# gddickinson/neural_enhanced_super_resolution

Measured on AMD Instinct MI355X. Metric: output megapixels/sec, RealESRGAN_x2plus x2 upscale, higher is better.
Workload: dtype f32 (operands as f16 hi+lo pairs, 3 f16 MFMAs per product, f32 accumulate); 1 GPU; c2: 512x512->1024x1024 RealESRGAN_x2plus fp32 single tile; frames_in_flight_per_gpu=1, world_size=1, partition=independent frames, no data-path collective

## Files before the change

neural_enhanced_super_resolution_amd/csrc/conv3x3_f16x2.hip:

```cpp
#include <cstdlib>
#include <type_traits>

#include "f16x2_common.h"
#include "nesr_kernels.h"

namespace nesr {


namespace {

constexpr int TW = 32, PW = TW + 2;
constexpr int WAVES = 4;
constexpr int RW = 2;

template <int DMAW>
struct Geo {
    static constexpr int LAUNCH_THREADS = 64 * (WAVES + DMAW);
    static constexpr int THREADS = 64 * (DMAW ? DMAW : WAVES);
    static constexpr int TH = WAVES * RW;
    static constexpr int PH = TH + 2;
    static constexpr int NPIX = PH * PW;
    static constexpr int IN_ITEMS = 4 * NPIX;
    static constexpr int IN_ROUNDS = (IN_ITEMS + THREADS - 1) / THREADS;
    static constexpr int IN_BYTES = IN_ITEMS * 16;
// ... 243 lines not shown
            const bool valid = X < a.w_ && Y < y_hi;
            const size_t pix = ((size_t)n * a.h + (Y < a.h ? Y : 0)) * a.w_ + (X < a.w_ ? X : 0);
            f32x4 v0, v1;
#pragma unroll
            for (int i = 0; i < 4; ++i) {
                const float e = fmaf(acc16[r][nh][0][1][i], LO_INV, acc16[r][nh][0][0][i]);
                const float o = fmaf(acc16[r][nh][1][1][i], LO_INV, acc16[r][nh][1][0][i]);
                const auto sw_ = __builtin_amdgcn_permlane16_swap(__float_as_uint(e), __float_as_uint(o), false, false);
                v0[i] = __uint_as_float(sw_[0]);
                v1[i] = __uint_as_float(sw_[1]);
            }
            v0 += bz0;
            v1 += bz1;
            if (a.lrelu) {
#pragma unroll
                for (int i = 0; i < 4; ++i) { v0[i] = fmaxf(v0[i], v0[i] * 0.2f); v1[i] = fmaxf(v1[i], v1[i] * 0.2f); }
            }
            auto slot = [&](const Map& mp, int coff) -> size_t { return (size_t)((coff + 32 * cg) >> 4) * mp.chunk + pix * mp.pix + piece8; };
            if (res1) {
                f32x4 q0, q1;
                load_regrouped(res1 + slot(a.res1_map, 0), a.res1_map.chunk, q0, q1);
#pragma unroll
                for (int i = 0; i < 4; ++i) { v0[i] = __fadd_rn(__fmul_rn(v0[i], a.s1), q0[i]); v1[i] = __fadd_rn(__fmul_rn(v1[i], a.s1), q1[i]); }
            }
            if (res2) {
                f32x4 q0, q1;
                load_regrouped(res2 + slot(a.res2_map, 0), a.res2_map.chunk, q0, q1);
#pragma unroll
                for (int i = 0; i < 4; ++i) { v0[i] = __fadd_rn(__fmul_rn(v0[i], a.s2), q0[i]); v1[i] = __fadd_rn(__fmul_rn(v1[i], a.s2), q1[i]); }
            }
            if (out || out2) {
                uint4 cx, cx1;
                bool bad_here = false;
                split_regroup(v0, v1, cx, cx1, bad_here);
                bad |= bad_here && valid;
                if (valid && out) {
                    uint16_t* p = out + slot(a.out_map, a.out_coff);
                    store16(p, cx);
                    store16(p + a.out_map.chunk, cx1);
                }
                if (valid && out2) {
                    uint16_t* p = out2 + slot(a.out2_map, 0);
                    store16(p, cx);
                    store16(p + a.out2_map.chunk, cx1);
                }
            }
            if (!valid) continue;
            if (a.cout_real > 0 && cb == 0) {
#pragma unroll
                for (int q = 0; q < 4; ++q) {
                    if (q >= a.cout_real) break;
                    const float x = poison ? __builtin_nanf("") : v0[q];
                    if (a.out_nchw) a.out_nchw[(((size_t)n * a.cout_real + q) * a.h + Y) * a.w_ + X] = x;
                    if (a.out_u8) {
                        float qv = fminf(fmaxf(x, 0.f), 1.f) * 255.0f;
                        qv = a.u8_round ? rintf(qv) : truncf(qv);
                        const int ch = a.u8_flip ? (a.cout_real - 1 - q) : q;
                        a.out_u8[pix * a.cout_real + ch] = (uint8_t)qv;
                    }
                }
            }
        }
    if (bad && a.status) __hip_atomic_store(a.status, 1u, __ATOMIC_RELAXED, __HIP_MEMORY_SCOPE_AGENT);
    STAMP(3);
#if NESR_ABL & 64
    asm volatile("s_waitcnt vmcnt(0)" ::: "memory");
    STAMP(4);
#endif
}

struct RdbArgs {
    const void* cur;
    long long chunk_bytes;
    void* out;
    const void* res2;
    float s1, s2;
    const void* w[5];
    const float* bias[5];
    int n, h, w_;
    unsigned* progress;
    unsigned epoch;
    unsigned* abort_flag;
    unsigned* status;
    unsigned long long timeout_ticks;
};

__device__ __forceinline__ void glds16_s_sc1(const char* sbase, unsigned voff, unsigned lds_dst) {
    unsigned keep;
    asm volatile(
        "s_mov_b32 %0, m0\n\t"
        "s_mov_b32 m0, %3\n\t"
        "s_nop 0\n\t"
        "global_load_lds_dwordx4 %1, %2 sc1\n\t"
        "s_mov_b32 m0, %0"
        : "=&s"(keep)
        : "v"(voff), "s"(sbase), "s"(lds_dst)
        : "memory");
}
__device__ __forceinline__ void store16_wt_s(const char* sbase, unsigned voff, uint4 v) {
    asm volatile("global_store_dwordx4 %0, %1, %2 sc1\n\ts_nop 1" ::"v"(voff), "v"(__builtin_bit_cast(f32x4, v)), "s"(sbase) : "memory");
}
__device__ __forceinline__ f32x4 load16_s(const char* sbase, unsigned voff) {
    return *(const __attribute__((address_space(1))) f32x4*)(sbase + voff);
}

#ifndef NESR_RDB_ABL
#define NESR_RDB_ABL 0
#endif

__device__ __forceinline__ void wait_vmcnt_le(int k) {
    switch (k) {
        case 0: asm volatile("s_waitcnt vmcnt(0)" ::: "memory"); break;
        case 1: asm volatile("s_waitcnt vmcnt(1)" ::: "memory"); break;
        case 2: asm volatile("s_waitcnt vmcnt(2)" ::: "memory"); break;
        case 3: asm volatile("s_waitcnt vmcnt(3)" ::: "memory"); break;
        case 4: asm volatile("s_waitcnt vmcnt(4)" ::: "memory"); break;
        case 5: asm volatile("s_waitcnt vmcnt(5)" ::: "memory"); break;
        case 6: asm volatile("s_waitcnt vmcnt(6)" ::: "memory"); break;
        case 7: asm volatile("s_waitcnt vmcnt(7)" ::: "memory"); break;
        case 8: asm volatile("s_waitcnt vmcnt(8)" ::: "memory"); break;
        case 9: asm volatile("s_waitcnt vmcnt(9)" ::: "memory"); break;
        case 10: asm volatile("s_waitcnt vmcnt(10)" ::: "memory"); break;
        case 11: asm volatile("s_waitcnt vmcnt(11)" ::: "memory"); break;
        default: asm volatile("s_waitcnt vmcnt(12)" ::: "memory"); break;
    }
}

#if NESR_RDB_ABL & 256
__device__ unsigned long long g_rdb_stamps[2][64][8];
__device__ unsigned long long g_rdb_taps[2][8][8];
__device__ unsigned long long g_rdb_arrive[12][8][2];
#define RARRIVE(w, step, ev) do { if (blockIdx.x == 77 && lane == 0 && (step) >= 20 && (step) < 28) { unsigned long long t_ = __builtin_amdgcn_s_memtime(); asm volatile("s_waitcnt lgkmcnt(0)" ::: "memory"); g_rdb_arrive[w][(step) - 20][ev] = t_; } } while (0)
#define RSTAMP(role, step, ev) do { if (blockIdx.x == 77 && lane == 0) { unsigned long long t_ = __builtin_amdgcn_s_memtime(); asm volatile("s_waitcnt lgkmcnt(0)" ::: "memory"); g_rdb_stamps[role][step][ev] = t_; } } while (0)
#else
#define RSTAMP(role, step, ev) do { } while (0)
#define RARRIVE(w, step, ev) do { } while (0)
#endif

constexpr int RSLOTS = 4;
constexpr int RDB_STEP5 = 4 + 6 + 8 + 10;
constexpr int RDB_STEPS = RDB_STEP5 + 12;
constexpr int W5_ROUNDS = 2 * W_ITEMS / (64 * 4);
static_assert(RSLOTS == 4 && RDB_STEP5 % RSLOTS == 0 && W5_ROUNDS * 64 * 4 == 2 * W_ITEMS, "conv5's slab pairs sit at ring positions 0,1 / 2,3 and fill whole DMA rounds");
constexpr int MW = 8;
constexpr int DW = 4;
#ifndef NESR_RDB_PAR
#define NESR_RDB_PAR 0
#endif
#ifndef NESR_RDB_EPI_STEPS
#define NESR_RDB_EPI_STEPS 1
#endif
constexpr int EPI_STEPS = NESR_RDB_EPI_STEPS;
static_assert(EPI_STEPS <= 4 - (RSLOTS - 1), "the tile would wait for its own progress word");

__global__ __launch_bounds__(64 * (MW + DW), 3) void rdb_f16x2_kernel(RdbArgs a) {
    typedef Geo<4> G;
    constexpr int THREADS = G::THREADS, TH = G::TH;
    constexpr int IN_ITEMS = G::IN_ITEMS, IN_ROUNDS = G::IN_ROUNDS, IN_BYTES = G::IN_BYTES;
    constexpr int W_ROUNDS = (W_ITEMS + THREADS - 1) / THREADS;
    constexpr int WRING = RSLOTS * IN_BYTES;
    constexpr int BIAS = RSLOTS * (IN_BYTES + W_BYTES);
    static_assert(TH == MW, "one tile row per MFMA wave");
    extern __shared__ __attribute__((aligned(16))) char smem[];

    const int lane = threadIdx.x & 63;
    const int wave_all = __builtin_amdgcn_readfirstlane(threadIdx.x >> 6);
    const bool is_dma = wave_all >= MW;
    const bool is_cmp = !is_dma;
    const int wave = is_cmp ? wave_all : wave_all - MW;
    const int tid = wave * 64 + lane;

    const int tiles_x = (a.w_ + TW - 1) / TW;
    const int tiles_y = (a.h + TH - 1) / TH;
    const int total = tiles_x * tiles_y * a.n;
    int tile;
    {
        const int bid = blockIdx.x, q = total >> 3, r = total & 7, xcd = bid & 7;
        tile = (xcd < r ? xcd * (q + 1) : r * (q + 1) + (xcd - r) * q) + (bid >> 3);
    }
    const int n = tile / (tiles_x * tiles_y);
    const int t2 = tile - n * tiles_x * tiles_y;
    const int ty = t2 / tiles_x, tx = t2 - ty * tiles_x;
    const int y0 = ty * TH, x0 = tx * TW;

    const int j16 = lane & 15, g4 = lane >> 4;
    auto advance = [](int& l, int& c) {
        const int nc = l == 4 ? 12 : 4 + 2 * l;
        if (++c == nc) { c = 0; ++l; }
    };

    if (is_dma) {
#ifdef NESR_RDB_DMAPRIO
        __builtin_amdgcn_s_setprio(NESR_RDB_DMAPRIO);
#endif
        if (wave == 0) RSTAMP(1, 61, 0);
        const unsigned lds_base = (unsigned)(size_t)(lds_char*)(smem);
        unsigned voff[IN_ROUNDS];
        unsigned okmask = 0;
        unsigned wavemask = 0;
        const int row0 = y0 > 0 ? y0 - 1 : 0;
        const char* in_img = static_cast<const char*>(a.cur) + ((size_t)n * a.h + row0) * a.w_ * 64;
        const unsigned* watch = nullptr;
        int kin = 0, kw = 0;
        if (lane < 9) {
            const int ny = ty + lane / 3 - 1, nx = tx + lane % 3 - 1;
            if (ny >= 0 && ny < tiles_y && nx >= 0 && nx < tiles_x) watch = a.progress + (n * tiles_y + ny) * tiles_x + nx;
        }
        {
            int p = tid >> 2;
            int py = p / PW, px = p - py * PW;
            const int sl = tid & 3;
#pragma unroll
            for (int i = 0; i < IN_ROUNDS; ++i) {
                const int k = tid + THREADS * i;
                const int sg = sl ^ (((px >> 2) & 1) << 1);
                const int Y = y0 - 1 + py, X = x0 - 1 + px;
                const bool has = k < IN_ITEMS;
                const bool ok = has && Y >= 0 && Y < a.h && X >= 0 && X < a.w_;
                voff[i] = ((unsigned)(Y - row0) * (unsigned)a.w_ + (unsigned)X) * 64u + sg * 16;
                okmask |= ok ? (1u << i) : 0u;
                if (__builtin_amdgcn_ballot_w64(ok) != 0ull) { wavemask |= 1u << i; ++kin; }
                if (has && !ok) {
#pragma unroll
                    for (int sl2 = 0; sl2 < RSLOTS; ++sl2) *reinterpret_cast<f32x4*>(smem + sl2 * IN_BYTES + k * 16) = f32x4{0.f, 0.f, 0.f, 0.f};
                }
                px += (THREADS / 4) % PW;
                py += (THREADS / 4) / PW;
                if (px >= PW) { px -= PW; py += 1; }
            }
#pragma unroll
            for (int j = 0; j < W_ROUNDS; ++j) kw += (wave * 64 + THREADS * j) < W_ITEMS ? 1 : 0;
        }
        unsigned seen = 0;
        bool gave_up = false;
        auto dma_w = [&](int l, int c, int wpos) {
            const char* wsrc = static_cast<const char*>(a.w[l]) + (size_t)c * W_BYTES;
#pragma unroll
            for (int j = 0; j < W_ROUNDS; ++j) {
                const int k = tid + THREADS * j;
                const unsigned dst = lds_base + WRING + wpos * W_BYTES + j * (THREADS * 16) + wave * 1024;
                if (k < W_ITEMS && !(NESR_RDB_ABL & 64)) glds16_s(wsrc, (unsigned)k * 16u, __builtin_amdgcn_readfirstlane(dst));
            }
        };
        auto dma_w5 = [&](int c, int wpos) {
            const char* wsrc = static_cast<const char*>(a.w[4]) + (size_t)c * (2 * W_BYTES);
#pragma unroll
            for (int j = 0; j < W5_ROUNDS; ++j) {
                const unsigned dst = lds_base + WRING + wpos * W_BYTES + j * (THREADS * 16) + wave * 1024;
                if (!(NESR_RDB_ABL & 64)) glds16_s(wsrc, (unsigned)(tid + THREADS * j) * 16u, __builtin_amdgcn_readfirstlane(dst));
            }
        };
        auto dma_in = [&](int c, int slot) {
            const unsigned need = c < 4 ? 0u : (unsigned)((c - 4) >> 1) + 1u;
            if (need > seen && !gave_up && !(NESR_RDB_ABL & 1)) {
                const unsigned target = a.epoch + need;
                unsigned long long t0 = 0;
                for (unsigned it = 0;; ++it) {
                    const unsigned v = watch ? __hip_atomic_load(watch, __ATOMIC_RELAXED, __HIP_MEMORY_SCOPE_AGENT) : target;
                    if (__builtin_amdgcn_ballot_w64((int)(v - target) < 0) == 0ull) break;
                    if ((it & 63u) == 0u) {
                        const unsigned long long now = __builtin_amdgcn_s_memrealtime();
                        if (it == 0) t0 = now;
                        const unsigned ab = __hip_atomic_load(a.abort_flag, __ATOMIC_RELAXED, __HIP_MEMORY_SCOPE_AGENT);
                        if (ab != 0u || now - t0 > a.timeout_ticks) {
                            if (ab == 0u && lane == 0) __hip_atomic_store(a.abort_flag, 1u | ((unsigned)c << 8) | ((unsigned)tile << 16), __ATOMIC_RELAXED, __HIP_MEMORY_SCOPE_AGENT);
                            gave_up = true;
                            break;
                        }
                    }
                    __builtin_amdgcn_s_sleep(4);
                }
                seen = need;
            }
            const char* isrc = in_img + (long long)c * a.chunk_bytes;
#pragma unroll
            for (int i = 0; i < IN_ROUNDS; ++i) {
                const unsigned dst = lds_base + slot * IN_BYTES + i * (THREADS * 16) + wave * 1024;
                if (((wavemask >> i) & 1u) && !(NESR_RDB_ABL & 32)) {
                    if ((okmask >> i) & 1u) {
                        if (NESR_RDB_ABL & 2) glds16_s(isrc, voff[i], __builtin_amdgcn_readfirstlane(dst));
                        else glds16_s_sc1(isrc, voff[i], __builtin_amdgcn_readfirstlane(dst));
                    }
                }
            }
        };
        int fl = 0, fc = 0;
#pragma unroll
        for (int i = 0; i < RSLOTS - 1; ++i) {
            dma_w(0, i, i);
            dma_in(i, i);
            advance(fl, fc);
        }
        gave_up = *(const __attribute__((address_space(4))) unsigned*)a.abort_flag != 0u;
        asm volatile("s_waitcnt lgkmcnt(0)" ::: "memory");
        int fill = 3;
        int cl = 0, cc = 0;
        wait_vmcnt_le((NESR_RDB_ABL & 96) ? 0 : 2 * (kw + kin));
        int inflight = kw + kin;
        __builtin_amdgcn_s_barrier();
        asm volatile("" ::: "memory");
        for (int step = 0; step < RDB_STEPS; ++step) {
            if (wave == 0) RSTAMP(1, step, 0);
#if NESR_RDB_ABL & 256
            if ((step == 0 || step == RDB_STEPS - 1) && wave == 0 && blockIdx.x == 77 && lane == 0) {
                const unsigned long long r_ = __builtin_amdgcn_s_memrealtime(), t_ = __builtin_amdgcn_s_memtime();
                asm volatile("s_waitcnt lgkmcnt(0)" ::: "memory");
                g_rdb_stamps[1][step == 0 ? 62 : 63][0] = r_;
                g_rdb_stamps[1][step == 0 ? 62 : 63][1] = t_;
            }
#endif
            wait_vmcnt_le((NESR_RDB_ABL & 96) ? 0 : inflight);
            if (wave == 0) RSTAMP(1, step, 1);
            RARRIVE(MW + wave, step, 0);
            if (!(NESR_RDB_ABL & 512)) __builtin_amdgcn_s_barrier();
            asm volatile("" ::: "memory");
            RARRIVE(MW + wave, step, 1);
            if (wave == 0) RSTAMP(1, step, 2);
            if (cc == EPI_STEPS && cl >= 1 && wave == 0 && lane == 0)
                __hip_atomic_store(a.progress + tile, a.epoch + (unsigned)cl, __ATOMIC_RELAXED, __HIP_MEMORY_SCOPE_AGENT);
            inflight = 0;
            if (step + 1 >= RDB_STEP5) {
                if (step + 1 < RDB_STEPS) dma_w5(step + 1 - RDB_STEP5, ((step + 1) & 1) * 2);
            } else if (fl < 4) {
                dma_w(fl, fc, (step + RSLOTS - 1) & (RSLOTS - 1));
                inflight += kw;
            }
            if (fl < 5) {
                dma_in(fc, fill);
                inflight += kin;
                advance(fl, fc);
                fill = fill == RSLOTS - 1 ? 0 : fill + 1;
            }
            if (wave == 0) RSTAMP(1, step, 3);
            advance(cl, cc);
        }
        return;
    }

#ifdef NESR_RDB_YPRIO
    if (wave >= 4) __builtin_amdgcn_s_setprio(NESR_RDB_YPRIO);
#endif
    const bool active = (y0 + wave) < a.h;
    if (wave == 1) RSTAMP(0, 61, 0);
    const bool fills_bias = wave < 6 && lane < 8;
    f32x4 bias_v = f32x4{0.f, 0.f, 0.f, 0.f};
    if (fills_bias) bias_v = *(const __attribute__((address_space(1))) f32x4*)(a.bias[wave < 4 ? wave : 4] + (wave == 5 ? 32 : 0) + 4 * lane);
    const int un = g4 >> 1, kh = g4 & 1;
    int b16[5][2], a16[5];
#pragma unroll
    for (int st_ = 0; st_ < 5; ++st_) {
        const int dy = st_ < 3 ? un : 2;
        const int dx = st_ < 3 ? st_ : (st_ == 3 ? un : 2);
#pragma unroll
        for (int nh = 0; nh < 2; ++nh) {
            const int col = 16 * nh + j16 + dx;
            b16[st_][nh] = ((wave + dy) * PW + col) * 64 + ((kh ^ (((col >> 2) & 1) << 1)) << 4);
        }
        a16[st_] = ((((dy * 3 + dx) * 2) * 2 + kh) * 32 + j16) * 16;
    }
    int slot = 0;
    int wpos = 0;
#if NESR_RDB_ABL & 256
    int mstep = 0;
#endif
    typedef const __attribute__((address_space(3))) f32x4* lds_f32x4;
    const unsigned lds0 = (unsigned)(size_t)(lds_char*)(smem);
    unsigned bcur[5], aw012, aw3, aw4, aw4b;
#pragma unroll
    for (int t = 0; t < 5; ++t) bcur[t] = lds0 + (unsigned)b16[t][0];
    const unsigned xl4 = (unsigned)((un ^ 1) << 5);
    aw012 = lds0 + (unsigned)(WRING + a16[0]);
    aw3 = lds0 + (unsigned)(WRING + a16[3]);
    aw4 = lds0 + (unsigned)(WRING + a16[4]);
    aw4b = aw4 + (unsigned)un * 1024u;
    const int par = (NESR_RDB_PAR >= 0) ? NESR_RDB_PAR : wave >> 2;
    const int cbl = (g4 & 1) * 16 + (g4 >> 1) * 8;
    const int piece8 = ((g4 & 1) * 2 + (g4 >> 1)) * 8;
    const bool res2 = a.res2 != nullptr;
    f32x4 ep[2][2];
#pragma unroll
    for (int nh = 0; nh < 2; ++nh)
#pragma unroll
        for (int mt = 0; mt < 2; ++mt) ep[nh][mt] = f32x4{0.f, 0.f, 0.f, 0.f};
    int ep_l = -1;
    bool bad = false;
    auto unpack_res = [&](f32x4 rx, f32x4 rx1, f32x4& q0, f32x4& q1) {
        uint4 cx = __builtin_bit_cast(uint4, rx), cx1 = __builtin_bit_cast(uint4, rx1);
        regroup_pairs(cx, cx1);
        const f16x8 h = __builtin_bit_cast(f16x8, cx), lo = __builtin_bit_cast(f16x8, cx1);
#pragma unroll
        for (int i = 0; i < 4; ++i) {
            q0[i] = fmaf((float)lo[i], LO_INV, (float)h[i]);
            q1[i] = fmaf((float)lo[4 + i], LO_INV, (float)h[4 + i]);
        }
    };
    const long long row_bytes = (((long long)n * a.h + (y0 + wave)) * a.w_) * 64;
    unsigned lane_off[2];
    bool lane_ok[2];
#pragma unroll
    for (int nh = 0; nh < 2; ++nh) {
        const int X = x0 + 16 * nh + j16;
        lane_ok[nh] = X < a.w_;
        lane_off[nh] = (unsigned)(lane_ok[nh] ? X : 0) * 64u + (unsigned)piece8 * 2u;
    }
    auto uni = [](const char* p) -> const char* {
        const unsigned long long v = (unsigned long long)p;
        const unsigned lo = __builtin_amdgcn_readfirstlane((unsigned)v), hi = __builtin_amdgcn_readfirstlane((unsigned)(v >> 32));
        return (const char*)(((unsigned long long)hi << 32) | lo);
    };
    auto epi_half = [&](int l, const f32x4& e0, const f32x4& e1, int nh) {
#if NESR_RDB_ABL & 256
        if (wave == 1) RSTAMP(0, mstep, 3);
#endif
        const bool valid = lane_ok[nh];
        const unsigned voff = lane_off[nh];
        const char* bsrc = smem + BIAS + (l * 32 + cbl) * 4;
        f32x4 v0, v1;
#pragma unroll
        for (int i = 0; i < 4; ++i) {
            const auto sw_ = __builtin_amdgcn_permlane16_swap(__float_as_uint(e0[i]), __float_as_uint(e1[i]), false, false);
            v0[i] = __uint_as_float(sw_[0]);
            v1[i] = __uint_as_float(sw_[1]);
        }
        v0 += *reinterpret_cast<const f32x4*>(bsrc);
        v1 += *reinterpret_cast<const f32x4*>(bsrc + 16);
        const int dchunk = 4 + 2 * l;
#pragma unroll
        for (int i = 0; i < 4; ++i) { v0[i] = fmaxf(v0[i], v0[i] * 0.2f); v1[i] = fmaxf(v1[i], v1[i] * 0.2f); }
#if NESR_RDB_ABL & 256
        asm volatile("" :: "v"(v0), "v"(v1));
        if (wave == 1) RSTAMP(0, mstep, 4);
#endif
        uint4 cx, cx1;
        bool bad_here = false;
        split_regroup(v0, v1, cx, cx1, bad_here);
        bad |= bad_here && valid;
#if NESR_RDB_ABL & 256
        asm volatile("" :: "v"(__builtin_bit_cast(f32x4, cx)), "v"(__builtin_bit_cast(f32x4, cx1)));
        if (wave == 1) RSTAMP(0, mstep, 5);
#endif
        if (valid) {
            const char* d0 = uni(static_cast<const char*>(a.cur) + (long long)dchunk * a.chunk_bytes + row_bytes);
            if (!(NESR_RDB_ABL & 4)) {
                store16_wt_s(d0, voff, cx);
                store16_wt_s(d0 + a.chunk_bytes, voff, cx1);
            } else {
                *reinterpret_cast<uint4*>(const_cast<char*>(d0) + voff) = cx;
                *reinterpret_cast<uint4*>(const_cast<char*>(d0) + a.chunk_bytes + voff) = cx1;
            }
        }
#if NESR_RDB_ABL & 256
        if (wave == 1) RSTAMP(0, mstep, 6);
#endif
    };
    auto epi_part = [&](int c) {
        if (NESR_RDB_ABL & 16) return;
        if (EPI_STEPS == 1) {
            epi_half(ep_l, ep[0][0], ep[0][1], 0);
            epi_half(ep_l, ep[1][0], ep[1][1], 1);
        } else if (c == 0) {
            epi_half(ep_l, ep[0][0], ep[0][1], 0);
        } else {
            epi_half(ep_l, ep[1][0], ep[1][1], 1);
        }
    };
    f32x4 R1[4][2], R2[4][2];
    auto issue_res = [&](const void* base, int g, f32x4 (&R)[4][2]) {
        const char* r = uni(static_cast<const char*>(base) + (long long)(2 * g) * a.chunk_bytes + row_bytes);
#pragma unroll
        for (int nh = 0; nh < 2; ++nh) {
            R[2 * g + nh][0] = load16_s(r, lane_off[nh]);
            R[2 * g + nh][1] = load16_s(r + a.chunk_bytes, lane_off[nh]);
        }
    };
    f32x4 acc16[2][2][2][2];
    f32x4 Af[2][2][2];
    f32x4 Bf[2][2][2];
    auto load_a = [&](int s_, int buf, unsigned off) {
#pragma unroll
        for (int mt = 0; mt < 2; ++mt) {
            if (s_ < 4) {
                const unsigned ad = s_ < 3 ? aw012 + s_ * 2048 : aw3;
                Af[buf][mt][0] = *((lds_f32x4)(size_t)(ad + off + mt * 256));
                Af[buf][mt][1] = *((lds_f32x4)(size_t)(ad + off + mt * 256 + 1024));
            } else {
                f32x4 hi = *((lds_f32x4)(size_t)(aw4 + off + mt * 256));
                Af[buf][mt][1] = *((lds_f32x4)(size_t)(aw4b + off + mt * 256));
                if (un) hi = f32x4{0.f, 0.f, 0.f, 0.f};
                Af[buf][mt][0] = hi;
            }
        }
    };
    auto move_a = [&](unsigned d) {
        aw012 += d;
        aw3 += d;
        aw4 += d;
        aw4b += d;
    };
    auto load_b = [&](int sl, int s_, int buf) {
        const unsigned dB = sl == RSLOTS - 1 ? (unsigned)(-(RSLOTS - 1) * IN_BYTES) : (unsigned)IN_BYTES;
        const unsigned xl = bcur[s_] ^ (s_ == 4 ? xl4 : 32u);
#pragma unroll
        for (int nh = 0; nh < 2; ++nh) {
            Bf[buf][nh][0] = *((lds_f32x4)(size_t)(bcur[s_] + nh * 1024));
            Bf[buf][nh][1] = *((lds_f32x4)(size_t)(xl + nh * 1024));
        }
        bcur[s_] += dB;
    };
    auto mfma_tap = [&](int s_, int g, int abuf, int bbuf) {
#pragma unroll
        for (int mt = 0; mt < 2; ++mt) {
            const f16x8 a0 = __builtin_bit_cast(f16x8, Af[abuf][mt][0]), a1 = __builtin_bit_cast(f16x8, Af[abuf][mt][1]);
#pragma unroll
            for (int nh = 0; nh < 2; ++nh) {
                const f16x8 x0_ = __builtin_bit_cast(f16x8, Bf[bbuf][nh][0]), x1_ = __builtin_bit_cast(f16x8, Bf[bbuf][nh][1]);
                if (s_ < 4) {
                    acc16[g][nh][mt][1] = __builtin_amdgcn_mfma_f32_16x16x32_f16(a0, x1_, acc16[g][nh][mt][1], 0, 0, 0);
                    acc16[g][nh][mt][0] = __builtin_amdgcn_mfma_f32_16x16x32_f16(a0, x0_, acc16[g][nh][mt][0], 0, 0, 0);
                    acc16[g][nh][mt][1] = __builtin_amdgcn_mfma_f32_16x16x32_f16(a1, x0_, acc16[g][nh][mt][1], 0, 0, 0);
                } else {
                    acc16[g][nh][mt][0] = __builtin_amdgcn_mfma_f32_16x16x32_f16(a0, x0_, acc16[g][nh][mt][0], 0, 0, 0);
                    acc16[g][nh][mt][1] = __builtin_amdgcn_mfma_f32_16x16x32_f16(a1, x1_, acc16[g][nh][mt][1], 0, 0, 0);
                }
            }
        }
    };
    auto zero_acc = [&](int g) {
#pragma unroll
        for (int nh = 0; nh < 2; ++nh)
#pragma unroll
            for (int mt = 0; mt < 2; ++mt)
#pragma unroll
                for (int q = 0; q < 2; ++q) acc16[g][nh][mt][q] = f32x4{0.f, 0.f, 0.f, 0.f};
    };
    auto step_body = [&](auto Pc, int c) {
        constexpr int P = decltype(Pc)::value;
        if (c == EPI_STEPS) asm volatile("s_waitcnt vmcnt(0)" ::: "memory");
#if NESR_RDB_ABL & 256
        if (wave == 1) RSTAMP(0, mstep, 0);
        RARRIVE(wave, mstep, 0);
#endif
        if (!(NESR_RDB_ABL & 512)) __builtin_amdgcn_s_barrier();
        asm volatile("" ::: "memory");
#if NESR_RDB_ABL & 256
        RARRIVE(wave, mstep, 1);
        if (wave == 1) RSTAMP(0, mstep, 1);
#endif
        const bool epi_now = active && ep_l >= 0 && c < EPI_STEPS;
        const int nslot = slot == RSLOTS - 1 ? 0 : slot + 1;
        const unsigned dA = wpos == RSLOTS - 1 ? (unsigned)(-(RSLOTS - 1) * W_BYTES) : (unsigned)W_BYTES;
        if (active && !(NESR_RDB_ABL & 8)) {
            if (epi_now && par == 0) {
                epi_part(c);
                __builtin_amdgcn_sched_barrier(0);
            }
#if NESR_RDB_ABL & 256
            unsigned long long tt[6];
#endif
#pragma unroll
            for (int s_ = 0; s_ < 5; ++s_) {
                const int buf = (s_ + P) & 1;
#if NESR_RDB_ABL & 256
                tt[s_] = __builtin_amdgcn_s_memtime();
                __builtin_amdgcn_sched_barrier(0);
#endif
                if (s_ + 1 < 5) {
                    load_a(s_ + 1, buf ^ 1, 0);
                    load_b(slot, s_ + 1, buf ^ 1);
                } else {
                    load_a(0, buf ^ 1, dA);
                    load_b(nslot, 0, buf ^ 1);
                }
                mfma_tap(s_, 0, buf, buf);
#pragma unroll
                for (int i = 0; i < 8; ++i) {
                    __builtin_amdgcn_sched_group_barrier(0x008, 1, 0);
                    __builtin_amdgcn_sched_group_barrier(0x100, 1, 0);
                }
                __builtin_amdgcn_sched_barrier(0);
            }
            if (epi_now && par == 1) {
                epi_part(c);
                __builtin_amdgcn_sched_barrier(0);
            }
#if NESR_RDB_ABL & 256
            tt[5] = __builtin_amdgcn_s_memtime();
            if (blockIdx.x == 77 && (wave == 1 || wave == 5) && lane == 0 && mstep >= 20 && mstep < 28) {
#pragma unroll
                for (int i = 0; i < 6; ++i) g_rdb_taps[wave == 5][mstep - 20][i] = tt[i];
            }
#endif
        }
        move_a(dA);
        slot = nslot;
        wpos = wpos == RSLOTS - 1 ? 0 : wpos + 1;
#if NESR_RDB_ABL & 256
        if (wave == 1) RSTAMP(0, mstep, 2);
        ++mstep;
#endif
    };
    auto step_body5 = [&](auto Pc, auto Fc, auto Lc, int c) {
        constexpr int P = decltype(Pc)::value;
        constexpr bool FIRST = decltype(Fc)::value == 1;
        constexpr bool last_of_all = decltype(Lc)::value != 0;
        if (c == EPI_STEPS) asm volatile("s_waitcnt vmcnt(0)" ::: "memory");
#if NESR_RDB_ABL & 256
        if (wave == 1) RSTAMP(0, mstep, 0);
        RARRIVE(wave, mstep, 0);
#endif
        if (!(NESR_RDB_ABL & 512)) __builtin_amdgcn_s_barrier();
        asm volatile("" ::: "memory");
#if NESR_RDB_ABL & 256
        RARRIVE(wave, mstep, 1);
        if (wave == 1) RSTAMP(0, mstep, 1);
#endif
        const bool epi_now = active && ep_l >= 0 && c < EPI_STEPS;
        const int nslot = slot == RSLOTS - 1 ? 0 : slot + 1;
        const unsigned dA = wpos == 0 ? (unsigned)(2 * W_BYTES) : (unsigned)(-2 * W_BYTES);
        if (active && !(NESR_RDB_ABL & 8)) {
            load_a(0, 0, 0);
            if (epi_now && par == 0) {
                epi_part(c);
                __builtin_amdgcn_sched_barrier(0);
            }
            if (FIRST) { zero_acc(0); zero_acc(1); }
#pragma unroll
            for (int s_ = 0; s_ < 5; ++s_) {
                const int buf = (s_ + P) & 1;
                if (last_of_all && s_ == 4 && !(NESR_RDB_ABL & 16)) {
                    issue_res(a.cur, 0, R1);
                    asm volatile("" ::: "memory");
                    __builtin_amdgcn_sched_barrier(0);
                }
                load_a(s_, 1, W_BYTES);
                if (s_ + 1 < 5) load_b(slot, s_ + 1, buf ^ 1);
                else if (!last_of_all) load_b(nslot, 0, buf ^ 1);
                mfma_tap(s_, 0, 0, buf);
#pragma unroll
                for (int i = 0; i < 8; ++i) {
                    __builtin_amdgcn_sched_group_barrier(0x008, 1, 0);
                    __builtin_amdgcn_sched_group_barrier(0x100, 1, 0);
                }
                __builtin_amdgcn_sched_barrier(0);
                if (s_ + 1 < 5) load_a(s_ + 1, 0, 0);
                else if (last_of_all && !(NESR_RDB_ABL & 16)) {
                    issue_res(a.cur, 1, R1);
                    asm volatile("" ::: "memory");
                    __builtin_amdgcn_sched_barrier(0);
                }
                mfma_tap(s_, 1, 1, buf);
                if (s_ + 1 < 5) {
#pragma unroll
                    for (int i = 0; i < 4; ++i) {
                        __builtin_amdgcn_sched_group_barrier(0x008, 2, 0);
                        __builtin_amdgcn_sched_group_barrier(0x100, 1, 0);
                    }
                }
                __builtin_amdgcn_sched_barrier(0);
            }
            if (epi_now && par == 1) {
                epi_part(c);
                __builtin_amdgcn_sched_barrier(0);
            }
        }
        move_a(dA);
        slot = nslot;
        wpos = wpos == 0 ? 2 : 0;
#if NESR_RDB_ABL & 256
        if (wave == 1) RSTAMP(0, mstep, 2);
        ++mstep;
#endif
    };
    if (fills_bias) *reinterpret_cast<f32x4*>(smem + BIAS + wave * 128 + lane * 16) = bias_v;
    asm volatile("s_waitcnt lgkmcnt(0)" ::: "memory");
    __builtin_amdgcn_s_barrier();
    asm volatile("" ::: "memory");
    if (active) {
        load_a(0, 0, 0);
        load_b(0, 0, 0);
    }
    typedef std::integral_constant<int, 0> I0;
    typedef std::integral_constant<int, 1> I1;
    for (int l = 0; l < 4; ++l) {
        const int nc = 4 + 2 * l;
        zero_acc(0);
        for (int c = 0; c < nc; c += 2) {
            step_body(I0{}, c);
            step_body(I1{}, c + 1);
        }
#pragma unroll
        for (int nh = 0; nh < 2; ++nh)
#pragma unroll
            for (int mt = 0; mt < 2; ++mt)
#pragma unroll
                for (int i = 0; i < 4; ++i) ep[nh][mt][i] = fmaf(acc16[0][nh][mt][1][i], LO_INV, acc16[0][nh][mt][0][i]);
        ep_l = l;
    }
    step_body5(I0{}, I1{}, I0{}, 0);
    step_body5(I1{}, I0{}, I0{}, 1);
    for (int c = 2; c < 10; c += 2) {
        step_body5(I0{}, I0{}, I0{}, c);
        step_body5(I1{}, I0{}, I0{}, c + 1);
    }
    step_body5(I0{}, I0{}, I0{}, 10);
    step_body5(I1{}, I0{}, I1{}, 11);
    auto final_epilogue = [&](auto Rc) {
        constexpr bool RES2 = decltype(Rc)::value != 0;
        if (RES2) {
            issue_res(a.res2, 0, R2);
            issue_res(a.res2, 1, R2);
        }
        asm volatile("" ::: "memory");
        __builtin_amdgcn_sched_barrier(0);
#if NESR_RDB_ABL & 256
        if (wave == 1) RSTAMP(0, mstep, 3);
#endif
        uint4 cx[4], cx1[4];
#pragma unroll
        for (int p = 0; p < 4; ++p) {
            const int g = p >> 1, nh = p & 1;
            f32x4 e0, e1;
#pragma unroll
            for (int i = 0; i < 4; ++i) {
                e0[i] = fmaf(acc16[g][nh][0][1][i], LO_INV, acc16[g][nh][0][0][i]);
                e1[i] = fmaf(acc16[g][nh][1][1][i], LO_INV, acc16[g][nh][1][0][i]);
            }
            const char* bsrc = smem + BIAS + (4 * 32 + 32 * g + cbl) * 4;
            f32x4 v0, v1;
#pragma unroll
            for (int i = 0; i < 4; ++i) {
                const auto sw_ = __builtin_amdgcn_permlane16_swap(__float_as_uint(e0[i]), __float_as_uint(e1[i]), false, false);
                v0[i] = __uint_as_float(sw_[0]);
                v1[i] = __uint_as_float(sw_[1]);
            }
            v0 += *reinterpret_cast<const f32x4*>(bsrc);
            v1 += *reinterpret_cast<const f32x4*>(bsrc + 16);
            f32x4 q0, q1;
            unpack_res(R1[p][0], R1[p][1], q0, q1);
#pragma unroll
            for (int i = 0; i < 4; ++i) { v0[i] = __fadd_rn(__fmul_rn(v0[i], a.s1), q0[i]); v1[i] = __fadd_rn(__fmul_rn(v1[i], a.s1), q1[i]); }
            if (RES2) {
                unpack_res(R2[p][0], R2[p][1], q0, q1);
#pragma unroll
                for (int i = 0; i < 4; ++i) { v0[i] = __fadd_rn(__fmul_rn(v0[i], a.s2), q0[i]); v1[i] = __fadd_rn(__fmul_rn(v1[i], a.s2), q1[i]); }
            }
            bool bad_here = false;
            split_regroup(v0, v1, cx[p], cx1[p], bad_here);
            bad |= bad_here && lane_ok[nh];
            __builtin_amdgcn_sched_barrier(0);
        }
#if NESR_RDB_ABL & 256
        if (wave == 1) RSTAMP(0, mstep, 5);
#endif
#pragma unroll
        for (int p = 0; p < 4; ++p) {
            if (lane_ok[p & 1]) {
                const char* d0 = uni(static_cast<const char*>(a.out) + (long long)(2 * (p >> 1)) * a.chunk_bytes + row_bytes);
                store16_wt_s(d0, lane_off[p & 1], cx[p]);
                store16_wt_s(d0 + a.chunk_bytes, lane_off[p & 1], cx1[p]);
            }
        }
#if NESR_RDB_ABL & 256
        if (wave == 1) RSTAMP(0, mstep, 6);
        asm volatile("s_waitcnt vmcnt(0)" ::: "memory");
        if (wave == 1) RSTAMP(0, 61, 1);
#endif
    };
    if (active && !(NESR_RDB_ABL & 16)) {
        if (res2) final_epilogue(I1{});
        else final_epilogue(I0{});
    }
    if (bad && a.status) __hip_atomic_store(a.status, 1u, __ATOMIC_RELAXED, __HIP_MEMORY_SCOPE_AGENT);
}

template <int DMAW, int NMT = 2>
hipError_t launch_split(const ConvArgs& a, hipStream_t s) {
    typedef Geo<DMAW> G;
    constexpr size_t shm = (size_t)ISLOTS * G::IN_BYTES + 2 * (size_t)W_BYTES;
    static unsigned long long attr_done = 0;
    {
        const hipError_t e = ensure_dynamic_lds(reinterpret_cast<const void*>(&conv3x3_f16x2_kernel<DMAW, NMT>), shm, attr_done);
        if (e != hipSuccess) return e;
    }
    const int rows = (a.y_hi > 0 ? a.y_hi : a.h) - a.y_lo;
    const long total = (long)((a.w_ + TW - 1) / TW) * ((rows + G::TH - 1) / G::TH) * a.n * (a.coutp / 32);
    if (total <= 0) return hipSuccess;
    if (total > 0x7fffffffL) return hipErrorInvalidValue;
    hipLaunchKernelGGL((conv3x3_f16x2_kernel<DMAW, NMT>), dim3((unsigned)total), dim3(G::LAUNCH_THREADS), shm, s, a);
    return hipGetLastError();
}


}

#if NESR_RDB_ABL & 256
extern "C" int nesr_debug_rdb_steps() { return RDB_STEPS; }
extern "C" int nesr_debug_rdb_stamps(unsigned long long* out) {
    return (int)hipMemcpyFromSymbol(out, HIP_SYMBOL(g_rdb_stamps), sizeof(unsigned long long) * 2 * 64 * 8);
}
extern "C" int nesr_debug_rdb_taps(unsigned long long* out) {
    return (int)hipMemcpyFromSymbol(out, HIP_SYMBOL(g_rdb_taps), sizeof(unsigned long long) * 2 * 8 * 8);
}
extern "C" int nesr_debug_rdb_arrive(unsigned long long* out) {
    return (int)hipMemcpyFromSymbol(out, HIP_SYMBOL(g_rdb_arrive), sizeof(unsigned long long) * 12 * 8 * 2);
}
#endif
#if NESR_ABL & 64
extern "C" int nesr_debug_stamps(unsigned long long* out, int n) {
    return (int)hipMemcpyFromSymbol(out, HIP_SYMBOL(g_stamps), sizeof(unsigned long long) * (n < 256 ? n : 256));
}
#endif

size_t packed_weight_elems_f16x2(int cin_p, int coutp) { return (size_t)cin_p * 9 * coutp * 2; }

void pack_weights_f16x2(const float* oihw, int cout, int cin, int cin_p, int coutp, uint16_t* dst) {
    const size_t total = packed_weight_elems_f16x2(cin_p, coutp);
    for (size_t i = 0; i < total; ++i) dst[i] = 0;
    const int groups = coutp / 32;
    for (int o = 0; o < cout; ++o)
        for (int ci = 0; ci < cin; ++ci)
            for (int tap = 0; tap < 9; ++tap) {
                const float wv = oihw[((size_t)o * cin + ci) * 9 + tap];
                const uint16_t hi = f2h(wv);
                const uint16_t lo = f2h((wv - h2f(hi)) * LO_SCALE);
                const int c = ci / 16, kh = (ci % 16) / 8, kk = ci % 8;
                const size_t slab = ((size_t)c * groups + o / 32) * (size_t)(W_ITEMS * 8);
                const size_t ihi = slab + ((((size_t)tap * 2 + 0) * 2 + kh) * 32 + o % 32) * 8 + kk;
                const size_t ilo = slab + ((((size_t)tap * 2 + 1) * 2 + kh) * 32 + o % 32) * 8 + kk;
                dst[ihi] = hi;
                dst[ilo] = lo;
            }
}

int rdb_f16x2_tiles(int n, int h, int w) { return ((w + TW - 1) / TW) * ((h + 7) / 8) * n; }

hipError_t launch_rdb_f16x2(const RdbLaunch& r, hipStream_t s) {
    typedef Geo<4> G;
    constexpr size_t shm = (size_t)RSLOTS * (G::IN_BYTES + (size_t)W_BYTES) + 768;
    static unsigned long long attr_done = 0;
    {
        const hipError_t e = ensure_dynamic_lds(reinterpret_cast<const void*>(&rdb_f16x2_kernel), shm, attr_done);
        if (e != hipSuccess) return e;
    }
    if ((long long)r.w_ * 64 * 12 >= (1ll << 32)) return hipErrorInvalidValue;
    RdbArgs a;
    a.cur = r.cur; a.chunk_bytes = r.chunk_bytes; a.out = r.out; a.res2 = r.res2; a.s1 = r.s1; a.s2 = r.s2;
    for (int i = 0; i < 5; ++i) { a.w[i] = r.w[i]; a.bias[i] = r.bias[i]; }
    a.n = r.n; a.h = r.h; a.w_ = r.w_;
    a.progress = r.progress; a.epoch = r.epoch; a.abort_flag = r.abort_flag; a.status = r.status;
// ... 40 lines not shown
```

Measured before the change: 170.7 MP/s.

## Stagger barrier placement for upper waves to overlap ring refill with taps

Introduces a lag mode where compute waves 4-7 take each step's workgroup barrier partway through the tap loop instead of at the step top, while waves 0-3 keep the leading schedule. The DMA waves' prefetch depth and per-step issue counts are recomputed from a constexpr walk that statically checks no ring slot is refilled while being read. The aim is to de-synchronise the compute waves so that barrier stalls and LDS/MFMA contention spread out, at the cost of one fewer ring slot of input lookahead and more complex scheduling.

Result: faster. 173.3 MP/s, median of 6 (+1.5%).

```diff
diff --git a/neural_enhanced_super_resolution_amd/csrc/conv3x3_f16x2.hip b/neural_enhanced_super_resolution_amd/csrc/conv3x3_f16x2.hip
--- a/neural_enhanced_super_resolution_amd/csrc/conv3x3_f16x2.hip
+++ b/neural_enhanced_super_resolution_amd/csrc/conv3x3_f16x2.hip
@@ -419,6 +419,125 @@
 #endif
 constexpr int EPI_STEPS = NESR_RDB_EPI_STEPS;
 static_assert(EPI_STEPS <= 4 - (RSLOTS - 1), "the tile would wait for its own progress word");
+
+#ifndef NESR_RDB_LAG
+#define NESR_RDB_LAG 2
+#endif
+namespace rdbs {
+constexpr int LAG = NESR_RDB_LAG;
+static_assert(LAG == 0 || LAG == 2 || LAG == 3, "NESR_RDB_LAG: 0, 2 (barrier in front of tap-step 3) or 3 (in front of tap-step 2)");
+constexpr int layer_of(int s) { return s < 4 ? 0 : s < 10 ? 1 : s < 18 ? 2 : s < RDB_STEP5 ? 3 : 4; }
+constexpr int first_of(int l) { return l == 0 ? 0 : l == 1 ? 4 : l == 2 ? 10 : l == 3 ? 18 : RDB_STEP5; }
+constexpr int steps_of(int l) { return l == 4 ? RDB_STEPS - RDB_STEP5 : 4 + 2 * l; }
+enum Mode {
+    M_TOP,
+    M_LEAD,
+    M_LAG_FIRST,
+    M_LAG_MID,
+    M_LAG_LAST,
+    M_CONV5
+};
+constexpr int mode_of(bool lagging, int s) {
+    const int l = layer_of(s), c = s - first_of(l);
+    return l == 4 ? M_CONV5 : LAG == 0 ? M_TOP : !lagging ? M_LEAD : c == 0 ? M_LAG_FIRST : c == steps_of(l) - 1 ? M_LAG_LAST : M_LAG_MID;
+}
+constexpr bool bar_top(int m) { return m != M_LAG_MID && m != M_LAG_LAST; }
+constexpr int bar_tap(int m) { return m == M_LAG_FIRST || m == M_LAG_MID ? 5 - LAG : -1; }
+constexpr bool req_behind(int m) { return m == M_LEAD || m == M_LAG_FIRST; }
+constexpr bool req_early(int m) { return m == M_TOP || m == M_LAG_FIRST || m == M_LAG_MID; }
+constexpr int in_end(int i) {
+    const int e = (LAG != 0 && i < RDB_STEP5) ? i + 3 : i + 4;
+    return e < RDB_STEPS ? e : RDB_STEPS;
+}
+constexpr int IN_LEAD = in_end(-1);
+constexpr bool w_slab(int i) { return i + 1 < RDB_STEP5 && in_end(i - 1) < RDB_STEP5; }
+constexpr bool w_pair(int i) { return i + 1 >= RDB_STEP5 && i + 1 < RDB_STEPS; }
+constexpr int tail_w(int i) { return w_slab(i) ? 1 : 0;}
+constexpr int tail_in(int i) {
+    const int n = in_end(i) - in_end(i - 1);
+    return LAG != 0 && i == RDB_STEP5 - 1 ? 0
+         : LAG != 0 && i == RDB_STEP5 ? 1
+         : n;
+}
+struct Walk {
+    int in_iss[RDB_STEPS] = {}, w_iss[RDB_STEPS] = {};
+    int in_land[RDB_STEPS] = {}, w_land[RDB_STEPS] = {};
+    int rd_lo[2][RDB_STEPS + 1] = {}, rd_hi[2][RDB_STEPS + 1] = {};
+    int wr_hi[2][RDB_STEPS + 1] = {};
+    int bars[3] = {};
+    bool ok = true;
+};
+constexpr bool pos_overlap_w(int t, int u) {
+    const int t0 = t < RDB_STEP5 ? (t & 3) : (t & 1) * 2, t1 = t < RDB_STEP5 ? t0 : t0 + 1;
+    const int u0 = u < RDB_STEP5 ? (u & 3) : (u & 1) * 2, u1 = u < RDB_STEP5 ? u0 : u0 + 1;
+    return t0 <= u1 && u0 <= t1;
+}
+constexpr Walk walk() {
+    Walk k;
+    for (int r = 0; r < 2; ++r) {
+        for (int i = 0; i <= RDB_STEPS; ++i) { k.rd_lo[r][i] = RDB_STEPS; k.rd_hi[r][i] = -1; k.wr_hi[r][i] = -1; }
+        int b = 1;
+        auto rd = [&](int t, bool pix, bool wts) {
+            if (t < k.rd_lo[r][b - 1]) k.rd_lo[r][b - 1] = t;
+            if (pix && t > k.rd_hi[r][b - 1]) k.rd_hi[r][b - 1] = t;
+            if (wts && t > k.wr_hi[r][b - 1]) k.wr_hi[r][b - 1] = t;
+        };
+        if (mode_of(r, 0) == M_TOP) rd(0, true, true);
+        for (int s = 0; s < RDB_STEPS; ++s) {
+            const int m = mode_of(r, s);
+            if (bar_top(m)) ++b;
+            for (int t = 0; t < 5; ++t) {
+                if (t == bar_tap(m)) ++b;
+                rd(s, true, true);
+                if (t == 4 && req_early(m)) rd(s + 1, true, s + 1 < RDB_STEP5);
+                if (t == 4 && m == M_CONV5 && s + 1 < RDB_STEPS) rd(s + 1, true, false);
+            }
+        }
+        k.bars[r] = b;
+    }
+    int q_step[3 * RDB_STEPS] = {}, q_w[3 * RDB_STEPS] = {}, qn = 0, landed = 0;
+    auto land = [&](int upto, int b) {
+        for (; landed < upto; ++landed) (q_w[landed] ? k.w_land : k.in_land)[q_step[landed]] = b;
+    };
+    for (int t = 0; t < IN_LEAD; ++t) {
+        q_step[qn] = t; q_w[qn++] = 1; k.w_iss[t] = -2;
+        q_step[qn] = t; q_w[qn++] = 0; k.in_iss[t] = -2;
+    }
+    land(qn - 2 * (IN_LEAD - 1), -1);
+    int tail = 2;
+    k.bars[2] = 1;
+    for (int i = 0; i < RDB_STEPS; ++i) {
+        land(qn - tail, i);
+        ++k.bars[2];
+        const int f = in_end(i - 1), e = in_end(i);
+        if (w_pair(i)) { q_step[qn] = i + 1; q_w[qn++] = 1; k.w_iss[i + 1] = i; }
+        else if (w_slab(i)) {
+            if (e - f != 1) k.ok = false;
+            q_step[qn] = f; q_w[qn++] = 1; k.w_iss[f] = i;
+        }
+        for (int t = f; t < e; ++t) { q_step[qn] = t; q_w[qn++] = 0; k.in_iss[t] = i; }
+        tail = tail_w(i) + tail_in(i);
+        if (tail_w(i) && tail_in(i) != e - f) k.ok = false;
+    }
+    if (qn != 2 * RDB_STEPS) k.ok = false;
+    land(qn, RDB_STEPS);
+    for (int r = 0; r < 2; ++r)
+        for (int i = -1; i < RDB_STEPS; ++i) {
+            for (int t = k.rd_lo[r][i + 1]; t <= k.rd_hi[r][i + 1]; ++t) {
+                if (k.in_land[t] > i) k.ok = false;
+                for (int u = t + 1; u < RDB_STEPS; ++u) if ((u & 3) == (t & 3) && k.in_iss[u] <= i) k.ok = false;
+            }
+            for (int t = k.rd_lo[r][i + 1]; t <= k.wr_hi[r][i + 1]; ++t) {
+                if (k.w_land[t] > i) k.ok = false;
+                for (int u = t + 1; u < RDB_STEPS; ++u) if (pos_overlap_w(t, u) && k.w_iss[u] <= i) k.ok = false;
+            }
+        }
+    return k;
+}
+constexpr Walk WALK = walk();
+static_assert(WALK.ok, "a ring position is refilled while it is read, or read before the wait that covers it");
+static_assert(WALK.bars[0] == RDB_STEPS + 1 && WALK.bars[1] == RDB_STEPS + 1 && WALK.bars[2] == RDB_STEPS + 1, "every role takes the same number of barriers");
+}
 
 __global__ __launch_bounds__(64 * (MW + DW), 3) void rdb_f16x2_kernel(RdbArgs a) {
     typedef Geo<4> G;
@@ -553,16 +672,16 @@
         };
         int fl = 0, fc = 0;
 #pragma unroll
-        for (int i = 0; i < RSLOTS - 1; ++i) {
+        for (int i = 0; i < rdbs::IN_LEAD; ++i) {
             dma_w(0, i, i);
             dma_in(i, i);
             advance(fl, fc);
         }
         gave_up = *(const __attribute__((address_space(4))) unsigned*)a.abort_flag != 0u;
         asm volatile("s_waitcnt lgkmcnt(0)" ::: "memory");
-        int fill = 3;
+        int fill = rdbs::IN_LEAD;
         int cl = 0, cc = 0;
-        wait_vmcnt_le((NESR_RDB_ABL & 96) ? 0 : 2 * (kw + kin));
+        wait_vmcnt_le((NESR_RDB_ABL & 96) ? 0 : (rdbs::IN_LEAD - 1) * (kw + kin));
         int inflight = kw + kin;
         __builtin_amdgcn_s_barrier();
         asm volatile("" ::: "memory");
@@ -585,19 +704,17 @@
             if (wave == 0) RSTAMP(1, step, 2);
             if (cc == EPI_STEPS && cl >= 1 && wave == 0 && lane == 0)
                 __hip_atomic_store(a.progress + tile, a.epoch + (unsigned)cl, __ATOMIC_RELAXED, __HIP_MEMORY_SCOPE_AGENT);
-            inflight = 0;
-            if (step + 1 >= RDB_STEP5) {
-                if (step + 1 < RDB_STEPS) dma_w5(step + 1 - RDB_STEP5, ((step + 1) & 1) * 2);
-            } else if (fl < 4) {
-                dma_w(fl, fc, (step + RSLOTS - 1) & (RSLOTS - 1));
-                inflight += kw;
-            }
-            if (fl < 5) {
+            if (rdbs::w_pair(step)) {
+                dma_w5(step + 1 - RDB_STEP5, ((step + 1) & 1) * 2);
+            } else if (rdbs::w_slab(step)) {
+                dma_w(fl, fc, fill);
+            }
+            for (int k = rdbs::in_end(step) - rdbs::in_end(step - 1); k > 0; --k) {
                 dma_in(fc, fill);
-                inflight += kin;
                 advance(fl, fc);
                 fill = fill == RSLOTS - 1 ? 0 : fill + 1;
             }
+            inflight = rdbs::tail_w(step) * kw + rdbs::tail_in(step) * kin;
             if (wave == 0) RSTAMP(1, step, 3);
             advance(cl, cc);
         }
@@ -800,23 +917,33 @@
 #pragma unroll
                 for (int q = 0; q < 2; ++q) acc16[g][nh][mt][q] = f32x4{0.f, 0.f, 0.f, 0.f};
     };
-    auto step_body = [&](auto Pc, int c) {
-        constexpr int P = decltype(Pc)::value;
-        if (c == EPI_STEPS) asm volatile("s_waitcnt vmcnt(0)" ::: "memory");
-#if NESR_RDB_ABL & 256
-        if (wave == 1) RSTAMP(0, mstep, 0);
-        RARRIVE(wave, mstep, 0);
-#endif
-        if (!(NESR_RDB_ABL & 512)) __builtin_amdgcn_s_barrier();
-        asm volatile("" ::: "memory");
-#if NESR_RDB_ABL & 256
-        RARRIVE(wave, mstep, 1);
-        if (wave == 1) RSTAMP(0, mstep, 1);
-#endif
+    auto step_body = [&](auto Pc, auto Mc, int c) {
+        constexpr int P = decltype(Pc)::value, M = decltype(Mc)::value;
+        constexpr int BT = rdbs::bar_tap(M);
+        auto bar = [&](int cb) {
+            if (cb == EPI_STEPS) asm volatile("s_waitcnt vmcnt(0)" ::: "memory");
+#if NESR_RDB_ABL & 256
+            if (wave == 1) RSTAMP(0, mstep, 0);
+            RARRIVE(wave, mstep + (cb - c), 0);
+#endif
+            if (!(NESR_RDB_ABL & 512)) __builtin_amdgcn_s_barrier();
+            asm volatile("" ::: "memory");
+#if NESR_RDB_ABL & 256
+            RARRIVE(wave, mstep + (cb - c), 1);
+            if (wave == 1) RSTAMP(0, mstep, 1);
+#endif
+        };
+        if (rdbs::bar_top(M)) bar(c);
         const bool epi_now = active && ep_l >= 0 && c < EPI_STEPS;
         const int nslot = slot == RSLOTS - 1 ? 0 : slot + 1;
         const unsigned dA = wpos == RSLOTS - 1 ? (unsigned)(-(RSLOTS - 1) * W_BYTES) : (unsigned)W_BYTES;
-        if (active && !(NESR_RDB_ABL & 8)) {
+        if (!(active && !(NESR_RDB_ABL & 8))) {
+            if (BT >= 0) bar(c + 1);
+        } else {
+            if (rdbs::req_behind(M)) {
+                load_a(0, P, 0);
+                load_b(slot, 0, P);
+            }
             if (epi_now && par == 0) {
                 epi_part(c);
                 __builtin_amdgcn_sched_barrier(0);
@@ -831,18 +958,24 @@
                 tt[s_] = __builtin_amdgcn_s_memtime();
                 __builtin_amdgcn_sched_barrier(0);
 #endif
+                if (s_ == BT) {
+                    bar(c + 1);
+                    __builtin_amdgcn_sched_barrier(0);
+                }
                 if (s_ + 1 < 5) {
                     load_a(s_ + 1, buf ^ 1, 0);
                     load_b(slot, s_ + 1, buf ^ 1);
-                } else {
+                } else if (rdbs::req_early(M)) {
                     load_a(0, buf ^ 1, dA);
                     load_b(nslot, 0, buf ^ 1);
                 }
                 mfma_tap(s_, 0, buf, buf);
-#pragma unroll
-                for (int i = 0; i < 8; ++i) {
-                    __builtin_amdgcn_sched_group_barrier(0x008, 1, 0);
-                    __builtin_amdgcn_sched_group_barrier(0x100, 1, 0);
+                if (s_ + 1 < 5 || rdbs::req_early(M)) {
+#pragma unroll
+                    for (int i = 0; i < 8; ++i) {
+                        __builtin_amdgcn_sched_group_barrier(0x008, 1, 0);
+                        __builtin_amdgcn_sched_group_barrier(0x100, 1, 0);
+                    }
                 }
                 __builtin_amdgcn_sched_barrier(0);
             }
@@ -886,6 +1019,7 @@
         const unsigned dA = wpos == 0 ? (unsigned)(2 * W_BYTES) : (unsigned)(-2 * W_BYTES);
         if (active && !(NESR_RDB_ABL & 8)) {
             load_a(0, 0, 0);
+            if (FIRST && !rdbs::req_early(rdbs::mode_of(false, RDB_STEP5 - 1))) load_b(slot, 0, P);
             if (epi_now && par == 0) {
                 epi_part(c);
                 __builtin_amdgcn_sched_barrier(0);
@@ -942,19 +1076,20 @@
     asm volatile("s_waitcnt lgkmcnt(0)" ::: "memory");
     __builtin_amdgcn_s_barrier();
     asm volatile("" ::: "memory");
-    if (active) {
+    if (active && rdbs::mode_of(false, 0) == rdbs::M_TOP) {
         load_a(0, 0, 0);
         load_b(0, 0, 0);
     }
     typedef std::integral_constant<int, 0> I0;
     typedef std::integral_constant<int, 1> I1;
-    for (int l = 0; l < 4; ++l) {
-        const int nc = 4 + 2 * l;
-        zero_acc(0);
-        for (int c = 0; c < nc; c += 2) {
-            step_body(I0{}, c);
-            step_body(I1{}, c + 1);
-        }
+    typedef std::integral_constant<int, rdbs::mode_of(false, 1)> MLead;
+    typedef std::integral_constant<int, rdbs::M_LAG_FIRST> MFirst;
+    typedef std::integral_constant<int, rdbs::M_LAG_MID> MMid;
+    typedef std::integral_constant<int, rdbs::M_LAG_LAST> MLast;
+    static_assert(rdbs::LAG == 0 || (rdbs::mode_of(true, 4) == rdbs::M_LAG_FIRST && rdbs::mode_of(true, 5) == rdbs::M_LAG_MID &&
+                                     rdbs::mode_of(true, 8) == rdbs::M_LAG_MID && rdbs::mode_of(true, 9) == rdbs::M_LAG_LAST &&
+                                     rdbs::mode_of(false, 0) == rdbs::mode_of(false, RDB_STEP5 - 1)), "the loops below are the walk's sequence");
+    auto layer_done = [&](int l) {
 #pragma unroll
         for (int nh = 0; nh < 2; ++nh)
 #pragma unroll
@@ -962,6 +1097,29 @@
 #pragma unroll
                 for (int i = 0; i < 4; ++i) ep[nh][mt][i] = fmaf(acc16[0][nh][mt][1][i], LO_INV, acc16[0][nh][mt][0][i]);
         ep_l = l;
+    };
+    if (rdbs::LAG == 0 || wave < 4) {
+        for (int l = 0; l < 4; ++l) {
+            const int nc = 4 + 2 * l;
+            zero_acc(0);
+            for (int c = 0; c < nc; c += 2) {
+                step_body(I0{}, MLead{}, c);
+                step_body(I1{}, MLead{}, c + 1);
+            }
+            layer_done(l);
+        }
+    } else {
+        for (int l = 0; l < 4; ++l) {
+            const int nc = 4 + 2 * l;
+            zero_acc(0);
+            step_body(I0{}, MFirst{}, 0);
+            for (int c = 1; c < nc - 1; c += 2) {
+                step_body(I1{}, MMid{}, c);
+                step_body(I0{}, MMid{}, c + 1);
+            }
+            step_body(I1{}, MLast{}, nc - 1);
+            layer_done(l);
+        }
     }
     step_body5(I0{}, I1{}, I0{}, 0);
     step_body5(I1{}, I0{}, I0{}, 1);
```
